# xjtu-omics/SVision

Hardware: AMD Instinct MI355X
Metric: candidate SV sites/sec (encode+CNN) (higher is better)
Workload: dtype f32

## Files before the change

include/svx.h:

```cpp
#ifndef SVX_H
#define SVX_H

#include <stdint.h>
#include <stddef.h>

#ifdef __cplusplus
extern "C" {
#endif

#define SVX_VERSION 420

#define SVX_OK            0
#define SVX_EINVAL       (-1)
#define SVX_ECAPACITY    (-2)
#define SVX_ELAUNCH      (-3)

#define SVX_IMG           227
#define SVX_LAYOUT_NHWC   0
#define SVX_LAYOUT_NCHW   1

#define SVX_GAP_INS       1
#define SVX_GAP_DEL       2

#define SVX_CONV_DENSE_PCT 97
// ... 44 lines not shown
int svx_fc_bias_act(const float* d_x, const float* d_w_packed, const float* d_bias, float* d_out, float* d_ws,
                    uint32_t m, uint32_t n, uint32_t k, int relu, void* stream);

int svx_fc8_softmax(const float* d_x, const float* d_w, const float* d_bias, float* d_out, uint32_t n, void* stream);

int svx_conv2d_same(const float* d_in, const float* d_w_packed, const float* d_bias, float* d_out, uint32_t n,
                    uint32_t cin, uint32_t cout, uint32_t height, uint32_t width, uint32_t ksize,
                    uint32_t groups, int relu, const int32_t* d_pixels, const uint32_t* d_pixel_count,
                    const float* d_background, void* stream);

int svx_image_dedup(const int32_t* d_records, uint32_t n, int32_t* d_unique, uint32_t* d_inv, uint32_t* d_live,
                    uint32_t* d_keys, uint32_t* d_ws, void* stream);

int svx_gather_rows(const float* d_src, const uint32_t* d_inv, float* d_dst, uint32_t n, uint32_t width, void* stream);

int svx_encode_conv1_live(const int32_t* d_records, uint32_t n, const float* d_w1, const float* d_base, float* d_y,
                          int lrn, uint32_t radius, float alpha, float beta, float k, uint32_t* d_touched,
                          const uint32_t* d_live, void* stream);
int svx_alexnet_active_sets_live(const uint32_t* d_touched, uint32_t n, int32_t* d_list2, int32_t* d_list3,
                                 int32_t* d_list4, int32_t* d_list5, uint32_t* d_counts, uint32_t* d_ws,
                                 uint64_t* d_totals, uint32_t* d_active2, const uint32_t* d_live, void* stream);
int svx_conv2d_same_live(const float* d_in, const float* d_w_packed, const float* d_bias, float* d_out, uint32_t n,
                         uint32_t cin, uint32_t cout, uint32_t height, uint32_t width, uint32_t ksize,
                         uint32_t groups, int relu, const int32_t* d_pixels, const uint32_t* d_pixel_count,
                         const float* d_background, const uint32_t* d_live, void* stream);
int svx_bias_relu_pool_lrn_live(const float* d_x, const float* d_bias, float* d_y, uint32_t n, uint32_t channels,
                                uint32_t height, uint32_t width, int lrn, uint32_t radius, float alpha, float beta,
                                float k, const uint32_t* d_active_rows, const float* d_background,
                                const uint32_t* d_live, void* stream);
int svx_fc_bias_act_live(const float* d_x, const float* d_w_packed, const float* d_bias, float* d_out, float* d_ws,
                         uint32_t m, uint32_t n, uint32_t k, int relu, const uint32_t* d_live, void* stream);
int svx_fc8_softmax_live(const float* d_x, const float* d_w, const float* d_bias, float* d_out, uint32_t n,
                         const uint32_t* d_live, void* stream);

int svx_span_position_distance(const double* d_start, const double* d_end, const uint64_t* d_part_off,
                               uint32_t n_parts, const uint64_t* d_out_off, uint64_t total_pairs,
                               double normalizer, double* d_out, void* stream);

typedef struct SvxHashJob {
    uint64_t x_off, y_off;
    uint32_t x_len, y_len;
    uint64_t table_off;
    uint32_t table_slots;
    uint32_t hit_cap;
    uint64_t hit_off;
} SvxHashJob;
int svx_hash_seeds(const uint8_t* d_bases, const SvxHashJob* d_jobs, uint32_t n_jobs, uint64_t* d_table,
                   int32_t* d_hits, uint32_t* d_counts, uint32_t k, uint32_t window, uint32_t max_x_len, void* stream);
int svx_hash_pack_hits(const SvxHashJob* d_jobs, uint32_t n_jobs, const int32_t* d_hits, const uint32_t* d_counts,
                       uint32_t* d_row_off, int32_t* d_packed, uint64_t packed_cap, void* stream);
size_t svx_hash_seeds_long_ws_bytes(uint32_t x_len, uint32_t y_len);
int svx_hash_seeds_long(const uint8_t* d_bases, const SvxHashJob* d_jobs, uint32_t n_jobs, uint64_t* d_table,
                        int32_t* d_hits, uint32_t* d_counts, void* d_ws, const uint64_t* d_ws_off,
                        uint32_t k, uint32_t window, uint32_t max_x_len, void* stream);

#define SVX_BAM_KEEP_SEQ 1
void*          svx_bam_open(const char* path, int threads, int flags);
void*          svx_bam_open_range(const char* path, int threads, int flags, uint64_t voff_beg, uint64_t voff_end);
const char*    svx_bam_error(void);
void           svx_bam_sizes(void* handle, uint64_t* sizes);
void           svx_bam_export(void* handle, int threads, int32_t* tid, int32_t* pos, uint16_t* flag, uint8_t* mapq,
                              int32_t* l_seq, int32_t* name_id, int64_t* cig_off, uint32_t* cigar, char* names,
                              char* header, char* ref_names, int32_t* ref_lens, int64_t* seq_off);
const uint8_t* svx_bam_seq(void* handle);
void           svx_bam_close(void* handle);

// ... 73 lines not shown
```

svision_amd/_lib.py:

```python
import ctypes
import os

_HERE = os.path.dirname(os.path.abspath(__file__))
LIB_PATH = os.path.join(_HERE, "libsvx.so")

SVX_OK = 0
SVX_EINVAL = -1
SVX_ECAPACITY = -2
SVX_ELAUNCH = -3
LAYOUT_NHWC = 0
LAYOUT_NCHW = 1
IMG = 227
GAP_INS = 1
GAP_DEL = 2

_vp, _u32, _i32, _u64, _sz = ctypes.c_void_p, ctypes.c_uint32, ctypes.c_int32, ctypes.c_uint64, ctypes.c_size_t
SYMBOLS = {
    "svx_version": (ctypes.c_int, []),
    "svx_strerror": (ctypes.c_char_p, [ctypes.c_int]),
    "svx_crc32c": (_u32, [_vp, _sz]),
    "svx_cigar_scan_ws_bytes": (_sz, [_u32, _u64]),
    "svx_cigar_scan": (ctypes.c_int, [_vp, _vp, _vp, _u32, _u64, _i32, _vp, _u64, _vp, _vp, _vp, _u64, _u32, _vp]),
    "svx_rasterize": (ctypes.c_int, [_vp, _u32, _vp, ctypes.c_int, ctypes.POINTER(ctypes.c_float), _vp]),
    "svx_encode_conv1": (ctypes.c_int, [_vp, _u32, _vp, _vp, _vp, ctypes.c_int, _u32, ctypes.c_float, ctypes.c_float,
                                        ctypes.c_float, _vp, _vp]),
    "svx_alexnet_active_sets": (ctypes.c_int, [_vp, _u32, _vp, _vp, _vp, _vp, _vp, _vp, _vp, _vp, _vp]),
    "svx_conv2d_same": (ctypes.c_int, [_vp, _vp, _vp, _vp, _u32, _u32, _u32, _u32, _u32, _u32, _u32, ctypes.c_int, _vp, _vp, _vp, _vp]),
    "svx_fc_ws_bytes": (_sz, [_u32, _u32, _u32]),
    "svx_fc_bias_act": (ctypes.c_int, [_vp, _vp, _vp, _vp, _vp, _u32, _u32, _u32, ctypes.c_int, _vp]),
    "svx_fc8_softmax": (ctypes.c_int, [_vp, _vp, _vp, _vp, _u32, _vp]),
    "svx_bias_relu_pool_lrn": (ctypes.c_int, [_vp, _vp, _vp, _u32, _u32, _u32, _u32, ctypes.c_int, _u32,
                                              ctypes.c_float, ctypes.c_float, ctypes.c_float, _vp, _vp, _vp]),
    "svx_image_dedup": (ctypes.c_int, [_vp, _u32, _vp, _vp, _vp, _vp, _vp, _vp]),
    "svx_gather_rows": (ctypes.c_int, [_vp, _vp, _vp, _u32, _u32, _vp]),
    "svx_encode_conv1_live": (ctypes.c_int, [_vp, _u32, _vp, _vp, _vp, ctypes.c_int, _u32, ctypes.c_float, ctypes.c_float,
                                             ctypes.c_float, _vp, _vp, _vp]),
    "svx_alexnet_active_sets_live": (ctypes.c_int, [_vp, _u32, _vp, _vp, _vp, _vp, _vp, _vp, _vp, _vp, _vp, _vp]),
    "svx_conv2d_same_live": (ctypes.c_int, [_vp, _vp, _vp, _vp, _u32, _u32, _u32, _u32, _u32, _u32, _u32, ctypes.c_int, _vp, _vp, _vp,
                                            _vp, _vp]),
    "svx_bias_relu_pool_lrn_live": (ctypes.c_int, [_vp, _vp, _vp, _u32, _u32, _u32, _u32, ctypes.c_int, _u32,
                                                   ctypes.c_float, ctypes.c_float, ctypes.c_float, _vp, _vp, _vp, _vp]),
    "svx_fc_bias_act_live": (ctypes.c_int, [_vp, _vp, _vp, _vp, _vp, _u32, _u32, _u32, ctypes.c_int, _vp, _vp]),
    "svx_fc8_softmax_live": (ctypes.c_int, [_vp, _vp, _vp, _vp, _u32, _vp, _vp]),
    "svx_span_position_distance":(ctypes.c_int, [_vp, _vp, _vp, _u32, _vp, _u64, ctypes.c_double, _vp, _vp]),
    "svx_hash_seeds": (ctypes.c_int, [_vp, _vp, _u32, _vp, _vp, _vp, _u32, _u32, _u32, _vp]),
    "svx_hash_pack_hits": (ctypes.c_int, [_vp, _u32, _vp, _vp, _vp, _vp, _u64, _vp]),
    "svx_hash_seeds_long_ws_bytes": (_sz, [_u32, _u32]),
    "svx_hash_seeds_long": (ctypes.c_int, [_vp, _vp, _u32, _vp, _vp, _vp, _vp, _vp, _u32, _u32, _u32, _vp]),
    "svx_bam_open": (_vp, [ctypes.c_char_p, ctypes.c_int, ctypes.c_int]),
    "svx_bam_open_range": (_vp, [ctypes.c_char_p, ctypes.c_int, ctypes.c_int, _u64, _u64]),
    "svx_bam_error": (ctypes.c_char_p, []),
    "svx_bam_sizes": (None, [_vp, _vp]),
    "svx_bam_export": (None, [_vp, ctypes.c_int] + [_vp] * 13),
    "svx_bam_seq": (_vp, [_vp]),
    "svx_bam_close": (None, [_vp]),
    "svx_bgzf_inflate_fast_ws_bytes": (_sz, [_u64, _u32]),
    "svx_bgzf_inflate_fast": (ctypes.c_int, [_vp, _vp, _vp, _vp, _u32, _u64, _vp, _vp, _vp, _u64, _vp]),
    "svx_bgzf_inflate_fast_on": (ctypes.c_int, [_vp, _vp, _vp, _vp, _u32, _u64, _vp, _vp, _vp, _u64, _vp, _vp]),
    "svx_bgzf_crc32": (ctypes.c_int, [_vp, _vp, _vp, _vp, _vp, _u32, _vp, _vp]),
    "svx_bam_walk_count": (ctypes.c_int, [_vp, _vp, _u32, _vp, _vp]),
    "svx_bam_walk_extract": (ctypes.c_int, [_vp, _vp, _u32, _vp] + [_vp] * 9 + [_u32, _vp]),
    "svx_bam_walk_count_seq": (ctypes.c_int, [_vp, _vp, _u32, _vp, _vp, _vp]),
    "svx_bam_walk_extract_seq": (ctypes.c_int, [_vp, _vp, _u32, _vp] + [_vp] * 12 + [_u32, _vp]),
    "svx_bam_find_starts_ws_bytes": (_sz, [_u32]),
    "svx_bam_find_starts": (ctypes.c_int, [_vp, _vp, _u32, _u64, _u32, _vp, _vp, _vp, _vp, _u64, _vp]),
    "svx_bam_walk_offsets": (ctypes.c_int, [_vp, _vp, _u32, _vp, _vp, _vp]),
    "svx_record_sort_ws_bytes": (_sz, [_u32]),
    "svx_record_sort": (ctypes.c_int, [_vp, _vp, _u32, _u32, _u32, _vp, _vp, _u64, _vp]),
    "svx_record_gather": (ctypes.c_int, [_vp, _vp, _vp, _u32, _u32, _vp]),
    "svx_record_gather_offsets_ws_bytes": (_sz, [_u32]),
    "svx_record_gather_offsets": (ctypes.c_int, [_vp, _vp, _u32, _vp, _vp, _u64, _vp]),
    "svx_record_gather_segments": (ctypes.c_int, [_vp, _vp, _vp, _vp, _vp, _u32, _u32, _vp]),
    "svx_record_invert": (ctypes.c_int, [_vp, _u32, _vp, _vp]),
    "svx_record_scatter_segments": (ctypes.c_int, [_vp, _vp, _vp, _u32, _u32, _vp, ctypes.c_int64, _vp, _u32, _vp, _vp]),
    "svx_bgzf_deflate": (ctypes.c_int, [_vp, _vp, _u32, _vp, _vp, _vp, _vp]),
    "svx_bgzf_deflate_dyn_ws_bytes": (_sz, [_u32]),
# ... 61 lines not shown
```

svision_amd/csrc/svx_cnn.hip:

```cpp
#include "svx_raster_common.hpp"

namespace {

constexpr int BLOCK = 256, WAVE = 64;

__device__ inline float lrn_scale(float v, float x, float beta)
{
    if (beta == 0.75f) return v * __frsqrt_rn(x) * __frsqrt_rn(__fsqrt_rn(x));
    return v / powf(x, beta);
}

__device__ inline float4 max4(float4 a, float4 b) { return make_float4(fmaxf(a.x, b.x), fmaxf(a.y, b.y), fmaxf(a.z, b.z), fmaxf(a.w, b.w)); }

__global__ __launch_bounds__(BLOCK)
void bias_relu_pool_lrn_kernel(const float* __restrict__ x, const float* __restrict__ bias, float* __restrict__ y,
                               int C, int H, int W, int OH, int OW, int lrn, int radius, float alpha, float beta, float k,
                               const uint32_t* __restrict__ active_rows, const float* __restrict__ background,
                               const uint32_t* __restrict__ live)
{
    extern __shared__ __attribute__((aligned(16))) float pooled[];
    const int b = blockIdx.x / OH;
    if (live && (uint32_t)b >= *live) return;
    const int oy = blockIdx.x - b * OH;
    const int CP = C + 1, HW = H * W;
// ... 350 lines not shown
    for (int p = t; p < 3 * A2 * A2; p += BLOCK) {
        const int l = p / (A2 * A2), q = p - l * (A2 * A2);
        const int y = q / A2, x = q - y * A2, r = A1 + l * A2 + y;
        const uint32_t m = masks[r], below = (1u << x) - 1u;
        const uint32_t slot = ((m >> x) & 1u) ? rowoff[r] + __popc(m & below) : inoff[r] + __popc(~m & below);
        ls[l][slot] = (int32_t)(img * (A2 * A2) + q);
    }
}
}

extern "C" int svx_alexnet_active_sets_live(const uint32_t* d_touched, uint32_t n, int32_t* d_list2, int32_t* d_list3,
                                            int32_t* d_list4, int32_t* d_list5, uint32_t* d_counts, uint32_t* d_ws,
                                            uint64_t* d_totals, uint32_t* d_active2, const uint32_t* d_live, void* stream)
{
    if (!d_counts) return SVX_EINVAL;
    hipStream_t st = static_cast<hipStream_t>(stream);
    if (n == 0) return hipMemsetAsync(d_counts, 0, 4 * sizeof(uint32_t), st) == hipSuccess ? SVX_OK : SVX_ELAUNCH;
    if (!d_touched || !d_list2 || !d_list3 || !d_list4 || !d_list5 || !d_ws || (reinterpret_cast<uintptr_t>(d_ws) & 15u)) return SVX_EINVAL;
    hipLaunchKernelGGL(active_counts_kernel, dim3(n), dim3(64), 0, st, d_touched, d_ws, d_live);
    hipLaunchKernelGGL(active_lists_kernel, dim3(n), dim3(BLOCK), 0, st, d_touched, d_ws, n, d_list2, d_list3, d_list4, d_list5, d_counts,
                       reinterpret_cast<unsigned long long*>(d_totals), d_active2, d_live);
    return hipGetLastError() == hipSuccess ? SVX_OK : SVX_ELAUNCH;
}

extern "C" int svx_alexnet_active_sets(const uint32_t* d_touched, uint32_t n, int32_t* d_list2, int32_t* d_list3,
                                       int32_t* d_list4, int32_t* d_list5, uint32_t* d_counts, uint32_t* d_ws,
                                       uint64_t* d_totals, uint32_t* d_active2, void* stream)
{
    return svx_alexnet_active_sets_live(d_touched, n, d_list2, d_list3, d_list4, d_list5, d_counts, d_ws, d_totals, d_active2, nullptr, stream);
}

namespace {
constexpr int FC8_IN = 4096, FC8_OUT = 5;
__global__ __launch_bounds__(64 * FC8_OUT)
void fc8_softmax_kernel(const float* __restrict__ x, const float* __restrict__ w, const float* __restrict__ bias,
                        float* __restrict__ out, const uint32_t* __restrict__ live)
{
    __shared__ float logit[FC8_OUT];
    const int img = blockIdx.x, cls = threadIdx.x >> 6, lane = threadIdx.x & 63;
    if (live && (uint32_t)img >= *live) return;
    const float4* xv = reinterpret_cast<const float4*>(x + (size_t)img * FC8_IN);
    const float4* wv = reinterpret_cast<const float4*>(w + (size_t)cls * FC8_IN);
    float acc = 0.0f;
#pragma unroll 4
    for (int i = lane; i < FC8_IN / 4; i += 64) {
        const float4 a = xv[i], b = wv[i];
        acc = fmaf(a.x, b.x, acc); acc = fmaf(a.y, b.y, acc); acc = fmaf(a.z, b.z, acc); acc = fmaf(a.w, b.w, acc);
    }
#pragma unroll
    for (int o = 32; o > 0; o >>= 1) acc += __shfl_xor(acc, o, 64);
    if (lane == 0) logit[cls] = acc + bias[cls];
    __syncthreads();
    if (threadIdx.x == 0) {
        float m = logit[0];
        int best = 0;
        for (int j = 1; j < FC8_OUT; ++j) if (logit[j] > m) { m = logit[j]; best = j; }
        float e[FC8_OUT], s = 0.0f;
        for (int j = 0; j < FC8_OUT; ++j) { e[j] = expf(logit[j] - m); s += e[j]; }
        float* o = out + (size_t)img * 12;
        for (int j = 0; j < FC8_OUT; ++j) { o[j] = e[j] / s; o[6 + j] = logit[j]; }
        o[5] = (float)best;
        o[11] = 0.0f;
    }
}
}

extern "C" int svx_fc8_softmax_live(const float* d_x, const float* d_w, const float* d_bias, float* d_out, uint32_t n,
                                    const uint32_t* d_live, void* stream)
{
    if (n == 0) return SVX_OK;
    if (!d_x || !d_w || !d_bias || !d_out) return SVX_EINVAL;
    if ((reinterpret_cast<uintptr_t>(d_x) & 15u) || (reinterpret_cast<uintptr_t>(d_w) & 15u)) return SVX_EINVAL;
    hipLaunchKernelGGL(fc8_softmax_kernel, dim3(n), dim3(64 * FC8_OUT), 0, static_cast<hipStream_t>(stream), d_x, d_w, d_bias, d_out, d_live);
    return hipGetLastError() == hipSuccess ? SVX_OK : SVX_ELAUNCH;
}

extern "C" int svx_fc8_softmax(const float* d_x, const float* d_w, const float* d_bias, float* d_out, uint32_t n, void* stream)
{
    return svx_fc8_softmax_live(d_x, d_w, d_bias, d_out, n, nullptr, stream);
}

extern "C" int svx_bias_relu_pool_lrn_live(const float* d_x, const float* d_bias, float* d_y, uint32_t n, uint32_t channels,
                                           uint32_t height, uint32_t width, int lrn, uint32_t radius, float alpha, float beta,
                                           float k, const uint32_t* d_active_rows, const float* d_background,
                                           const uint32_t* d_live, void* stream)
{
    if (n == 0) return SVX_OK;
    if (!d_x || !d_bias || !d_y || channels == 0 || channels % 8 || height < 3 || width < 3) return SVX_EINVAL;
    if ((reinterpret_cast<uintptr_t>(d_x) | reinterpret_cast<uintptr_t>(d_bias) | reinterpret_cast<uintptr_t>(d_y)) & 15u) return SVX_EINVAL;
    if ((d_active_rows == nullptr) != (d_background == nullptr) || (reinterpret_cast<uintptr_t>(d_background) & 15u) || (d_active_rows && width > 32)) return SVX_EINVAL;
    const int OH = (int)(height - 3) / 2 + 1, OW = (int)(width - 3) / 2 + 1;
    const size_t lds = (size_t)(channels + 1) * OW * sizeof(float);
    if (lds > 64 * 1024) return SVX_EINVAL;
    hipLaunchKernelGGL(bias_relu_pool_lrn_kernel, dim3(n * OH), dim3(BLOCK), lds, static_cast<hipStream_t>(stream),
                       d_x, d_bias, d_y, (int)channels, (int)height, (int)width, OH, OW, lrn, (int)radius, alpha, beta, k,
                       d_active_rows, d_background, d_live);
    return hipGetLastError() == hipSuccess ? SVX_OK : SVX_ELAUNCH;
// ... 10 lines not shown
```

svision_amd/csrc/svx_dedup.hip:

```cpp
#include "svx_raster_common.hpp"

namespace {

constexpr int KEY_BLOCK = 256, COMPACT_BLOCK = 1024, WAVE = 64;

__device__ inline bool key_eq(const uint4& a, const uint4& b) { return a.x == b.x && a.y == b.y && a.z == b.z && a.w == b.w; }

__global__ __launch_bounds__(KEY_BLOCK)
void first_kernel(const int32_t* __restrict__ records, uint32_t n, uint32_t* __restrict__ first, uint4* __restrict__ keys)
{
    __shared__ uint4 tile[KEY_BLOCK];
    const uint32_t i = blockIdx.x * KEY_BLOCK + threadIdx.x;
    const uint4 mine = i < n ? svx_raster::image_key(records + (size_t)i * 12) : uint4{0, 0, 0, 0};
    if (keys && i < n) keys[i] = mine;
    uint32_t f = i;
    for (uint32_t t = 0; t <= blockIdx.x; ++t) {
        const uint32_t j0 = t * KEY_BLOCK;
        __syncthreads();
        if (t == blockIdx.x) tile[threadIdx.x] = mine;
        else tile[threadIdx.x] = svx_raster::image_key(records + (size_t)(j0 + threadIdx.x) * 12);
        __syncthreads();
        if (f == i) {
            const uint32_t hi = min((uint32_t)KEY_BLOCK, i - j0);
            for (uint32_t j = 0; j < hi; ++j)
                if (key_eq(tile[j], mine)) { f = j0 + j; break; }
        }
    }
    if (i < n) first[i] = f;
}

__global__ __launch_bounds__(COMPACT_BLOCK)
void compact_kernel(const int32_t* __restrict__ records, uint32_t n, uint32_t* __restrict__ inv, uint32_t* __restrict__ row,
                    int32_t* __restrict__ unique, uint32_t* __restrict__ live)
{
    __shared__ uint32_t wave_sum[COMPACT_BLOCK / WAVE];
    __shared__ uint32_t s_base;
    const int t = threadIdx.x, lane = t & (WAVE - 1), wv = t / WAVE;
    if (t == 0) s_base = 0;
    __syncthreads();
    for (uint32_t c0 = 0; c0 < n; c0 += COMPACT_BLOCK) {
        const uint32_t i = c0 + t;
        const bool is_first = i < n && inv[i] == i;
        const unsigned long long ball = __ballot(is_first);
        const uint32_t below = __popcll(ball & ((1ull << lane) - 1ull));
        if (lane == 0) wave_sum[wv] = __popcll(ball);
        __syncthreads();
        uint32_t before = s_base;
        for (int w = 0; w < wv; ++w) before += wave_sum[w];
        if (is_first) {
            const uint32_t c = before + below;
            row[i] = c;
#pragma unroll
            for (int e = 0; e < 12; ++e) unique[(size_t)c * 12 + e] = records[(size_t)i * 12 + e];
        }
        __syncthreads();
        if (t == 0) { uint32_t s = s_base; for (int w = 0; w < COMPACT_BLOCK / WAVE; ++w) s += wave_sum[w]; s_base = s; }
        __syncthreads();
    }
    const uint32_t n_live = s_base;
    for (uint32_t e = n_live * 12 + t; e < n * 12; e += COMPACT_BLOCK) unique[e] = records[e % 12];
    for (uint32_t i = t; i < n; i += COMPACT_BLOCK) inv[i] = row[inv[i]];
    if (t == 0) *live = n_live;
}

__global__ __launch_bounds__(256)
void gather_rows_kernel(const float* __restrict__ src, const uint32_t* __restrict__ inv, float* __restrict__ dst, uint32_t n, uint32_t width)
{
    const uint32_t e = blockIdx.x * 256 + threadIdx.x;
    if (e >= n * width) return;
    const uint32_t i = e / width, c = e - i * width;
    dst[e] = src[(size_t)inv[i] * width + c];
}

}

extern "C" int svx_image_dedup(const int32_t* d_records, uint32_t n, int32_t* d_unique, uint32_t* d_inv, uint32_t* d_live,
                               uint32_t* d_keys, uint32_t* d_ws, void* stream)
{
    if (!d_live) return SVX_EINVAL;
    hipStream_t st = static_cast<hipStream_t>(stream);
    if (n == 0) return hipMemsetAsync(d_live, 0, sizeof(uint32_t), st) == hipSuccess ? SVX_OK : SVX_ELAUNCH;
    if (!d_records || !d_unique || !d_inv || !d_ws || n > (1u << 26)) return SVX_EINVAL;
    if (reinterpret_cast<uintptr_t>(d_keys) & 15u) return SVX_EINVAL;
    hipLaunchKernelGGL(first_kernel, dim3((n + KEY_BLOCK - 1) / KEY_BLOCK), dim3(KEY_BLOCK), 0, st, d_records, n, d_inv,
                       reinterpret_cast<uint4*>(d_keys));
    hipLaunchKernelGGL(compact_kernel, dim3(1), dim3(COMPACT_BLOCK), 0, st, d_records, n, d_inv, d_ws, d_unique, d_live);
    return hipGetLastError() == hipSuccess ? SVX_OK : SVX_ELAUNCH;
}

extern "C" int svx_gather_rows(const float* d_src, const uint32_t* d_inv, float* d_dst, uint32_t n, uint32_t width, void* stream)
{
    if (n == 0 || width == 0) return SVX_OK;
    if (!d_src || !d_inv || !d_dst || (uint64_t)n * width > 0xffffffffull) return SVX_EINVAL;
    const uint32_t total = n * width;
    hipLaunchKernelGGL(gather_rows_kernel, dim3((total + 255) / 256), dim3(256), 0, static_cast<hipStream_t>(stream), d_src, d_inv, d_dst, n, width);
    return hipGetLastError() == hipSuccess ? SVX_OK : SVX_ELAUNCH;
}
```

svision_amd/csrc/svx_fc.hip:

```cpp
#include <hip/hip_runtime.h>
#include <stdint.h>
#include "../../include/svx.h"
#include "svx_shadow.hpp"

namespace {

typedef float v16f __attribute__((ext_vector_type(16)));
typedef float v4f __attribute__((ext_vector_type(4)));
constexpr int THREADS = 256, WAVES = THREADS / 64;

__device__ __forceinline__ v4f buf_load4(__amdgpu_buffer_rsrc_t rsrc, unsigned voff, unsigned soff)
{
    return __builtin_bit_cast(v4f, __builtin_amdgcn_raw_buffer_load_b128(rsrc, (int)voff, (int)soff, 0));
}

#ifndef SVX_FC_RING_A
#define SVX_FC_RING_A 6
#endif

template <int U> struct StageIndex { static constexpr int value = U; };

template <int N, int U = 0, typename F>
__device__ __forceinline__ void svx_unroll_stages(F& f)
{
    if constexpr (U < N) { f(StageIndex<U>{}); svx_unroll_stages<N, U + 1>(f); }
}

template <int N, int U = 0, typename F>
__device__ __forceinline__ void svx_tail_stages(F& f, int left)
{
    if constexpr (U < N - 1) {
        if (left > U) { f(StageIndex<U>{}); svx_tail_stages<N, U + 1>(f, left); }
    }
}

struct FcArgs { const float* x; const float* w; float* part; int M, N, K, splits; const uint32_t* live; };

template <int NA, int NB>
__global__ __launch_bounds__(THREADS, 2)
void fc_splitk_kernel(const FcArgs a)
{
    SVX_SHADOW_ROOM();
    const int n_tiles = a.N / (32 * NA), m_tiles = (a.M + 32 * NB - 1) / (32 * NB);
    const int total = m_tiles * a.splits * n_tiles;
    const int wt = blockIdx.x * WAVES + (threadIdx.x >> 6);
    if (wt >= total) return;
    const int nt = wt % n_tiles, rest = wt / n_tiles;
    const int s = rest % a.splits, mt = rest / a.splits;
    const int m_live = a.live ? min((int)*a.live, a.M) : a.M;
    if (mt * 32 * NB >= m_live) return;
    const int lane = threadIdx.x & 63, hi = lane >> 5, lo = lane & 31;
    const int KQ = a.K / 8;
    const int q0 = (int)((long long)KQ * s / a.splits), q1 = (int)((long long)KQ * (s + 1) / a.splits);
    const __amdgpu_buffer_rsrc_t rs_w = __builtin_amdgcn_make_buffer_rsrc(const_cast<float*>(a.w), 0, (int)((long long)a.N * a.K * 4), 0x00020000);
    const __amdgpu_buffer_rsrc_t rs_x = __builtin_amdgcn_make_buffer_rsrc(const_cast<float*>(a.x), 0, (int)((long long)a.M * a.K * 4), 0x00020000);
    unsigned voff_a[NA], voff_b[NB];
#pragma unroll
    for (int i = 0; i < NA; ++i) voff_a[i] = (unsigned)((((nt * NA + i) * KQ + q0) * 32 + lo) * 32 + 16 * hi);
#pragma unroll
    for (int t = 0; t < NB; ++t) voff_b[t] = (unsigned)(((mt * NB + t) * 32 + lo) * a.K * 4 + (q0 * 8 + 4 * hi) * 4);
    v16f acc[NA][NB];
#pragma unroll
    for (int i = 0; i < NA; ++i)
#pragma unroll
        for (int t = 0; t < NB; ++t)
#pragma unroll
            for (int r = 0; r < 16; ++r) acc[i][t][r] = 0.0f;
    constexpr int RA = SVX_FC_RING_A, RB = 3, MF = 4 * NA * NB, L = NA + NB;
    static_assert(RA % RB == 0, "weight ring must be a multiple of the activation ring");
    v4f ra[RA][NA], rb[RB][NB];
    unsigned soff_a = 0, soff_b = 0;
    auto load_a = [&](int slot) {
#pragma unroll
        for (int i = 0; i < NA; ++i) ra[slot][i] = buf_load4(rs_w, voff_a[i], soff_a);
        soff_a += 1024u;
    };
    auto load_b1 = [&](int slot, int t) { rb[slot][t] = buf_load4(rs_x, voff_b[t], soff_b); };
    auto stage = [&](auto u_) {
        constexpr int u = decltype(u_)::value;
        constexpr int sa = u % RA, sb = u % RB, la = (u + RA - 1) % RA, lb = (u + RB - 1) % RB;
#pragma unroll
        for (int m = 0; m < MF; ++m) {
            if (m == 0) load_a(la);
#pragma unroll
            for (int t = 0; t < NB; ++t)
                if ((t + 1) * MF / L == m) load_b1(lb, t);
            const int j = m / (NA * NB), r = m - j * (NA * NB);
            const int i = r / NB, t = r - i * NB;
            acc[i][t] = __builtin_amdgcn_mfma_f32_32x32x2f32(ra[sa][i][j], rb[sb][t][j], acc[i][t], 0, 0, 0);
            __builtin_amdgcn_sched_barrier(0);
        }
        soff_b += 32u;
    };
    const int Q = q1 - q0;
#pragma unroll
    for (int p = 0; p < RA - 1; ++p) load_a(p);
#pragma unroll
    for (int p = 0; p < RB - 1; ++p) {
#pragma unroll
        for (int t = 0; t < NB; ++t) load_b1(p, t);
        soff_b += 32u;
    }
    __builtin_amdgcn_sched_barrier(0);
    const int QU = Q - Q % RA;
    for (int q = 0; q < QU; q += RA) svx_unroll_stages<RA>(stage);
    svx_tail_stages<RA>(stage, Q - QU);
#pragma unroll
    for (int i = 0; i < NA; ++i)
#pragma unroll
        for (int t = 0; t < NB; ++t) {
            const int m = (mt * NB + t) * 32 + lo;
            if (m >= m_live) continue;
            float* o = a.part + ((size_t)s * a.M + m) * a.N + (nt * NA + i) * 32 + 4 * hi;
#pragma unroll
            for (int u = 0; u < 4; ++u)
                *reinterpret_cast<v4f*>(o + 8 * u) = v4f{acc[i][t][4 * u], acc[i][t][4 * u + 1], acc[i][t][4 * u + 2], acc[i][t][4 * u + 3]};
        }
}

__global__ __launch_bounds__(THREADS)
void fc_reduce_kernel(const float* __restrict__ part, const float* __restrict__ bias, float* __restrict__ out, int MN4, int N4, int splits, int relu,
                      const uint32_t* __restrict__ live)
{
    const int e = blockIdx.x * THREADS + threadIdx.x;
    if (e >= MN4 || (live && (uint32_t)(e / N4) >= *live)) return;
    const float4* p = reinterpret_cast<const float4*>(part);
    float4 v = reinterpret_cast<const float4*>(bias)[e % N4];
    for (int s = 0; s < splits; ++s) { const float4 q = p[(size_t)s * MN4 + e]; v.x += q.x; v.y += q.y; v.z += q.z; v.w += q.w; }
    if (relu) { v.x = fmaxf(v.x, 0.0f); v.y = fmaxf(v.y, 0.0f); v.z = fmaxf(v.z, 0.0f); v.w = fmaxf(v.w, 0.0f); }
    reinterpret_cast<float4*>(out)[e] = v;
}

int fc_na(uint32_t m, uint32_t n)
{
    int na = (m > 64 && n % 64 == 0) ? 2 : 1;
#ifdef SVX_CONV_EXPERIMENT
    if (const char* e = getenv("SVX_FC_NA")) if (atoi(e) == 1 || (atoi(e) == 2 && m > 32 && n % 64 == 0)) na = atoi(e);
#endif
    return na;
}

int fc_splits(uint32_t m, uint32_t n, uint32_t k)
{
    const int tiles = (int)(n / (32 * fc_na(m, n))) * (int)((m + 63) / 64);
    int s = (1024 + tiles - 1) / tiles;
    const int max_s = (int)(k / 8) / 24;
    if (s > max_s) s = max_s;
#ifdef SVX_CONV_EXPERIMENT
    if (const char* e = getenv("SVX_FC_SPLITS")) if (atoi(e) >= 1 && atoi(e) <= max_s) s = atoi(e);
#endif
    return s < 1 ? 1 : s;
}

}

extern "C" size_t svx_fc_ws_bytes(uint32_t m, uint32_t n, uint32_t k)
{
    return (size_t)fc_splits(m, n, k) * m * n * sizeof(float);
}

extern "C" int svx_fc_bias_act_live(const float* d_x, const float* d_w_packed, const float* d_bias, float* d_out, float* d_ws,
                                    uint32_t m, uint32_t n, uint32_t k, int relu, const uint32_t* d_live, void* stream)
{
    if (m == 0) return SVX_OK;
    if (!d_x || !d_w_packed || !d_bias || !d_out || !d_ws || n % 32 || k % 8 || k < 24 * 8) return SVX_EINVAL;
    for (const void* p : {(const void*)d_x, (const void*)d_w_packed, (const void*)d_bias, (const void*)d_out, (const void*)d_ws})
        if (reinterpret_cast<uintptr_t>(p) & 15u) return SVX_EINVAL;
    if ((uint64_t)n * k * 4 > 0x7fffffffull || (uint64_t)m * k * 4 > 0x7fffffffull) return SVX_EINVAL;
    hipStream_t st = static_cast<hipStream_t>(stream);
    FcArgs a{d_x, d_w_packed, d_ws, (int)m, (int)n, (int)k, fc_splits(m, n, k), d_live};
    const int m_tiles = (int)((m + 63) / 64);
    const int na = fc_na(m, n);
    const int waves = m_tiles * a.splits * (int)(n / (32 * na));
    const dim3 grid((unsigned)((waves + WAVES - 1) / WAVES));
    if (na == 2)      hipLaunchKernelGGL((fc_splitk_kernel<2, 2>), grid, dim3(THREADS), 0, st, a);
    else if (m <= 32) hipLaunchKernelGGL((fc_splitk_kernel<1, 1>), grid, dim3(THREADS), 0, st, a);
    else              hipLaunchKernelGGL((fc_splitk_kernel<1, 2>), grid, dim3(THREADS), 0, st, a);
    const int mn4 = (int)((uint64_t)m * n / 4);
    hipLaunchKernelGGL(fc_reduce_kernel, dim3((mn4 + THREADS - 1) / THREADS), dim3(THREADS), 0, st, d_ws, d_bias, d_out, mn4, (int)(n / 4), a.splits, relu, d_live);
    return hipGetLastError() == hipSuccess ? SVX_OK : SVX_ELAUNCH;
}

extern "C" int svx_fc_bias_act(const float* d_x, const float* d_w_packed, const float* d_bias, float* d_out, float* d_ws,
                               uint32_t m, uint32_t n, uint32_t k, int relu, void* stream)
{
    return svx_fc_bias_act_live(d_x, d_w_packed, d_bias, d_out, d_ws, m, n, k, relu, nullptr, stream);
}
```

svision_amd/kernels.py:

```python
import ctypes

import numpy as np
import torch

from . import _lib

GAP_DTYPE = np.dtype([("aln", "<u4"), ("op", "<u4"), ("read_pos", "<i4"),
                      ("ref_pos", "<i4"), ("len", "<i4"), ("kind", "<u4")])
MEAN = (104.0, 117.0, 124.0)


def to_c8(x):
    n, c, h, w = x.shape
    if c % 8:
        raise _lib.SvxError("the C8 layout needs a channel count that is a multiple of 8")
    return x.reshape(n, c // 8, 8, h, w).permute(0, 1, 3, 4, 2).contiguous()


def from_c8(x):
    n, o, h, w, e = x.shape
    return x.permute(0, 1, 4, 2, 3).reshape(n, o * e, h, w).contiguous()


def pack_conv_weights(w_hwio):
# ... 252 lines not shown
def fc_bias_act(x, w_packed, bias, relu=True, out=None, ws=None, live=None):
    lib = _lib.load()
    for t, nm in ((x, "x"), (w_packed, "w_packed"), (bias, "bias")):
        _require_cuda(t, nm)
    if x.dtype != torch.float32 or x.dim() != 2 or w_packed.dim() != 4 or w_packed.shape[2:] != (32, 8) or w_packed.shape[1] * 8 != x.shape[1]:
        raise _lib.SvxError("x must be float32 [m,k] and w packed [n/32,k/8,32,8]")
    m, k = x.shape
    n = w_packed.shape[0] * 32
    if bias.numel() != n:
        raise _lib.SvxError("bias must have n entries")
    if out is None:
        out = torch.empty((m, n), dtype=torch.float32, device=x.device)
    need = lib.svx_fc_ws_bytes(m, n, k)
    if ws is None or ws.numel() * ws.element_size() < need:
        ws = torch.empty(max(need, 16) // 4, dtype=torch.float32, device=x.device)
    rc = lib.svx_fc_bias_act_live(x.data_ptr(), w_packed.data_ptr(), bias.data_ptr(), out.data_ptr(), ws.data_ptr(), m, n, k,
                                  1 if relu else 0, _check_live(live), _stream_ptr(x.device))
    _lib.check(rc, "svx_fc_bias_act")
    return out


def fc8_softmax(x, w_out_in, bias, out=None, live=None):
    lib = _lib.load()
    for t, nm in ((x, "x"), (w_out_in, "w"), (bias, "bias")):
        _require_cuda(t, nm)
    if x.dtype != torch.float32 or x.dim() != 2 or x.shape[1] != 4096 or tuple(w_out_in.shape) != (5, 4096):
        raise _lib.SvxError("x must be float32 [n,4096] and w float32 [5,4096]")
    n = x.shape[0]
    if out is None:
        out = torch.empty((n, 12), dtype=torch.float32, device=x.device)
    rc = lib.svx_fc8_softmax_live(x.data_ptr(), w_out_in.data_ptr(), bias.data_ptr(), out.data_ptr(), n, _check_live(live),
                                  _stream_ptr(x.device))
    _lib.check(rc, "svx_fc8_softmax")
    return out


def span_position_distance(starts, ends, part_off, normalizer=1000.0):
    lib = _lib.load()
    _require_cuda(starts, "starts")
    _require_cuda(ends, "ends")
    if starts.dtype != torch.float64 or ends.dtype != torch.float64 or starts.numel() != ends.numel():
        raise _lib.SvxError("starts / ends must be float64 tensors of one length")
    part = np.ascontiguousarray(part_off, np.uint64)
    if part.ndim != 1 or part.size < 1 or int(part[-1]) != starts.numel() or np.any(np.diff(part.astype(np.int64)) < 0):
        raise _lib.SvxError("part_off must be ascending and end at the number of signatures")
    sizes = np.diff(part.astype(np.int64))
    out_off = np.zeros(part.size, np.uint64)
    out_off[1:] = np.cumsum(sizes * (sizes - 1) // 2)
    total = int(out_off[-1])
    out = torch.empty(total, dtype=torch.float64, device=starts.device)
    if total:
        d_part = torch.from_numpy(part.view(np.int64)).to(starts.device)
        d_off = torch.from_numpy(out_off.view(np.int64)).to(starts.device)
        rc = lib.svx_span_position_distance(starts.data_ptr(), ends.data_ptr(), d_part.data_ptr(), part.size - 1, d_off.data_ptr(), total,
                                            float(normalizer), out.data_ptr(), _stream_ptr(starts.device))
        _lib.check(rc, "svx_span_position_distance")
    return out, out_off


HASH_MAX_X = 2048
HASH_LONG_MAX_X = 65536
_BASE_CODE = np.full(256, 255, np.uint8)
for _i, _c in enumerate(b"ACGTNacgtnRYKMS"):
    _BASE_CODE[_c] = _i
HASH_JOB_DTYPE = np.dtype([("x_off", "<u8"), ("y_off", "<u8"), ("x_len", "<u4"), ("y_len", "<u4"), ("table_off", "<u8"),
                           ("table_slots", "<u4"), ("hit_cap", "<u4"), ("hit_off", "<u8")])
# ... 454 lines not shown
```

svision_amd/network/alexnet.py:

```python
import numpy as np
import torch

CLASSES = ("DEL", "INS", "INV", "DUP", "tDUP")

_CONVS = (
    ("conv1", 11, 3, 96, 4, 0, 1),
    ("conv2", 5, 48, 256, 1, 2, 2),
    ("conv3", 3, 256, 384, 1, 1, 1),
    ("conv4", 3, 192, 384, 1, 1, 2),
    ("conv5", 3, 192, 256, 1, 1, 2),
)
_FCS = (("fc6", 9216, 4096), ("fc7", 4096, 4096), ("fc8", 4096, 5))


def checkpoint_shapes():
    shapes = {}
    for name, k, cin, cout, _s, _p, _g in _CONVS:
        shapes[f"{name}/weights"] = (k, k, cin, cout)
        shapes[f"{name}/biases"] = (cout,)
    for name, nin, nout in _FCS:
        shapes[f"{name}/weights"] = (nin, nout)
        shapes[f"{name}/biases"] = (nout,)
    return shapes

# ... 101 lines not shown
    @torch.no_grad()
    def background(self):
        if self._background is None:
            from .. import kernels
            from .create_batch import PAD_DATA, parse_data_fields
            dev = self.conv1_base.device
            rec = torch.tensor([parse_data_fields(PAD_DATA.split("_"))], dtype=torch.int32, device=dev)
            x1, touched = kernels.encode_conv1(rec, self.conv1_hwio, self.conv1_base, touched=True)
            rows = touched[0].cpu().numpy().astype("int64") & ((1 << 27) - 1)
            free = [(y, x) for y in range(27) for x in range(27) if not (int(rows[y]) >> x) & 1]
            if not free:
                raise RuntimeError("the padding record touches every pooled pixel")
            c = x1[0, :, free[0][0], free[0][1], :]
            x = c.reshape(1, 12, 1, 1, 8).expand(1, 12, 27, 27, 8).contiguous()
            bg = {}
            bg["conv2"] = kernels.conv2d_same(x, self.conv2_w, None, groups=2)
            x = kernels.bias_relu_pool_lrn(bg["conv2"], self.conv2_b, lrn=True)
            bg["conv3"] = kernels.conv2d_same(x, self.conv3_w, self.conv3_b, groups=1, relu=True)
            bg["conv4"] = kernels.conv2d_same(bg["conv3"], self.conv4_w, self.conv4_b, groups=2, relu=True)
            bg["conv5"] = kernels.conv2d_same(bg["conv4"], self.conv5_w, None, groups=2)
            self._background = bg
        return self._background

    @torch.no_grad()
    def predict_records_packed(self, records, out=None, memo=None):
        from .. import kernels
        memo = self.memo if memo is None else bool(memo)
        live = inv = None
        if memo and records.shape[0] > 0:
            records, inv, live = kernels.image_dedup(records)
        x = self._convs(records, live)
        x = x.reshape(x.shape[0], 9216)
        x = kernels.fc_bias_act(x, self.fc6_w, self.fc6_b, relu=True, live=live)
        x = kernels.fc_bias_act(x, self.fc7_w, self.fc7_b, relu=True, live=live)
        if live is None:
            return kernels.fc8_softmax(x, self.fc8_w, self.fc8_b, out=out)
        packed = kernels.fc8_softmax(x, self.fc8_w, self.fc8_b, live=live)
        return kernels.gather_rows(packed, inv, out=out)

    @torch.no_grad()
    def predict_records(self, records):
        packed = self.predict_records_packed(records)
        return packed[:, 6:11], packed[:, 5].to(torch.int64), packed[:, :5]
```

Measured before the change: 7779.

## Fuse fc7 reduce, fc8 softmax and row gather; add small-batch dedup and live FC path

On the memoized path, fc7's split-K reduce, bias and ReLU are folded into a new fc8 tail kernel. That kernel also computes the softmax and scatters results to duplicate rows through the inverse map, which replaces three launches. Deduplication gets a single-block kernel for batches of at most one compact block, skipping the separate first-occurrence pass. The FC split-K kernel gets a live-count-aware variant that picks narrow tiles when few unique rows survive. The risks are an O(n) scan of inv per block in the tail kernel, and a quadratic key comparison in the small dedup kernel.

```diff
diff --git a/include/svx.h b/include/svx.h
--- a/include/svx.h
+++ b/include/svx.h
@@ -100,6 +100,12 @@
                          uint32_t m, uint32_t n, uint32_t k, int relu, const uint32_t* d_live, void* stream);
 int svx_fc8_softmax_live(const float* d_x, const float* d_w, const float* d_bias, float* d_out, uint32_t n,
                          const uint32_t* d_live, void* stream);
+
+uint32_t svx_fc_splits(uint32_t m, uint32_t n, uint32_t k);
+int svx_fc_partial_live(const float* d_x, const float* d_w_packed, float* d_ws, uint32_t m, uint32_t n, uint32_t k,
+                        const uint32_t* d_live, void* stream);
+int svx_fc8_tail_live(const float* d_part, uint32_t splits, const float* d_bias7, const float* d_w, const float* d_bias,
+                      const uint32_t* d_inv, float* d_out, uint32_t m, uint32_t n, const uint32_t* d_live, void* stream);
 
 int svx_span_position_distance(const double* d_start, const double* d_end, const uint64_t* d_part_off,
                                uint32_t n_parts, const uint64_t* d_out_off, uint64_t total_pairs,
diff --git a/svision_amd/_lib.py b/svision_amd/_lib.py
--- a/svision_amd/_lib.py
+++ b/svision_amd/_lib.py
@@ -42,6 +42,9 @@
                                                    ctypes.c_float, ctypes.c_float, ctypes.c_float, _vp, _vp, _vp, _vp]),
     "svx_fc_bias_act_live": (ctypes.c_int, [_vp, _vp, _vp, _vp, _vp, _u32, _u32, _u32, ctypes.c_int, _vp, _vp]),
     "svx_fc8_softmax_live": (ctypes.c_int, [_vp, _vp, _vp, _vp, _u32, _vp, _vp]),
+    "svx_fc_splits": (_u32, [_u32, _u32, _u32]),
+    "svx_fc_partial_live": (ctypes.c_int, [_vp, _vp, _vp, _u32, _u32, _u32, _vp, _vp]),
+    "svx_fc8_tail_live": (ctypes.c_int, [_vp, _u32, _vp, _vp, _vp, _vp, _vp, _u32, _u32, _vp, _vp]),
     "svx_span_position_distance":(ctypes.c_int, [_vp, _vp, _vp, _u32, _vp, _u64, ctypes.c_double, _vp, _vp]),
     "svx_hash_seeds": (ctypes.c_int, [_vp, _vp, _u32, _vp, _vp, _vp, _u32, _u32, _u32, _vp]),
     "svx_hash_pack_hits": (ctypes.c_int, [_vp, _u32, _vp, _vp, _vp, _vp, _u64, _vp]),
diff --git a/svision_amd/csrc/svx_cnn.hip b/svision_amd/csrc/svx_cnn.hip
--- a/svision_amd/csrc/svx_cnn.hip
+++ b/svision_amd/csrc/svx_cnn.hip
@@ -406,14 +406,9 @@
 
 namespace {
 constexpr int FC8_IN = 4096, FC8_OUT = 5;
-__global__ __launch_bounds__(64 * FC8_OUT)
-void fc8_softmax_kernel(const float* __restrict__ x, const float* __restrict__ w, const float* __restrict__ bias,
-                        float* __restrict__ out, const uint32_t* __restrict__ live)
-{
-    __shared__ float logit[FC8_OUT];
-    const int img = blockIdx.x, cls = threadIdx.x >> 6, lane = threadIdx.x & 63;
-    if (live && (uint32_t)img >= *live) return;
-    const float4* xv = reinterpret_cast<const float4*>(x + (size_t)img * FC8_IN);
+__device__ __forceinline__ void fc8_row(const float4* xv, const float* __restrict__ w, const float* __restrict__ bias, float* logit, float* o)
+{
+    const int cls = threadIdx.x >> 6, lane = threadIdx.x & 63;
     const float4* wv = reinterpret_cast<const float4*>(w + (size_t)cls * FC8_IN);
     float acc = 0.0f;
 #pragma unroll 4
@@ -422,7 +417,7 @@
         acc = fmaf(a.x, b.x, acc); acc = fmaf(a.y, b.y, acc); acc = fmaf(a.z, b.z, acc); acc = fmaf(a.w, b.w, acc);
     }
 #pragma unroll
-    for (int o = 32; o > 0; o >>= 1) acc += __shfl_xor(acc, o, 64);
+    for (int d = 32; d > 0; d >>= 1) acc += __shfl_xor(acc, d, 64);
     if (lane == 0) logit[cls] = acc + bias[cls];
     __syncthreads();
     if (threadIdx.x == 0) {
@@ -431,12 +426,59 @@
         for (int j = 1; j < FC8_OUT; ++j) if (logit[j] > m) { m = logit[j]; best = j; }
         float e[FC8_OUT], s = 0.0f;
         for (int j = 0; j < FC8_OUT; ++j) { e[j] = expf(logit[j] - m); s += e[j]; }
-        float* o = out + (size_t)img * 12;
         for (int j = 0; j < FC8_OUT; ++j) { o[j] = e[j] / s; o[6 + j] = logit[j]; }
         o[5] = (float)best;
         o[11] = 0.0f;
     }
 }
+
+__global__ __launch_bounds__(64 * FC8_OUT)
+void fc8_softmax_kernel(const float* __restrict__ x, const float* __restrict__ w, const float* __restrict__ bias,
+                        float* __restrict__ out, const uint32_t* __restrict__ live)
+{
+    __shared__ float logit[FC8_OUT];
+    const int img = blockIdx.x;
+    if (live && (uint32_t)img >= *live) return;
+    fc8_row(reinterpret_cast<const float4*>(x + (size_t)img * FC8_IN), w, bias, logit, out + (size_t)img * 12);
+}
+
+__global__ __launch_bounds__(64 * FC8_OUT)
+void fc8_tail_kernel(const float* __restrict__ part, const float* __restrict__ bias7, const float* __restrict__ w, const float* __restrict__ bias,
+                     const uint32_t* __restrict__ inv, float* __restrict__ out, uint32_t m, uint32_t n, int splits, const uint32_t* __restrict__ live)
+{
+    __shared__ float4 xs[FC8_IN / 4];
+    __shared__ float logit[FC8_OUT];
+    __shared__ float packed[12];
+    const uint32_t img = blockIdx.x;
+    if (live && img >= *live) return;
+    const size_t mn4 = (size_t)m * (FC8_IN / 4);
+    const float4* p = reinterpret_cast<const float4*>(part) + (size_t)img * (FC8_IN / 4);
+    for (int i = threadIdx.x; i < FC8_IN / 4; i += 64 * FC8_OUT) {
+        float4 v = reinterpret_cast<const float4*>(bias7)[i];
+        for (int s = 0; s < splits; ++s) { const float4 q = p[(size_t)s * mn4 + i]; v.x += q.x; v.y += q.y; v.z += q.z; v.w += q.w; }
+        v.x = fmaxf(v.x, 0.0f); v.y = fmaxf(v.y, 0.0f); v.z = fmaxf(v.z, 0.0f); v.w = fmaxf(v.w, 0.0f);
+        xs[i] = v;
+    }
+    __syncthreads();
+    fc8_row(xs, w, bias, logit, packed);
+    __syncthreads();
+    for (uint32_t i = threadIdx.x; i < n; i += 64 * FC8_OUT)
+        if (inv[i] == img) {
+#pragma unroll
+            for (int e = 0; e < 12; ++e) out[(size_t)i * 12 + e] = packed[e];
+        }
+}
+}
+
+extern "C" int svx_fc8_tail_live(const float* d_part, uint32_t splits, const float* d_bias7, const float* d_w, const float* d_bias,
+                                 const uint32_t* d_inv, float* d_out, uint32_t m, uint32_t n, const uint32_t* d_live, void* stream)
+{
+    if (m == 0 || n == 0) return SVX_OK;
+    if (!d_part || !d_bias7 || !d_w || !d_bias || !d_inv || !d_out || splits == 0) return SVX_EINVAL;
+    if ((reinterpret_cast<uintptr_t>(d_part) | reinterpret_cast<uintptr_t>(d_bias7) | reinterpret_cast<uintptr_t>(d_w)) & 15u) return SVX_EINVAL;
+    hipLaunchKernelGGL(fc8_tail_kernel, dim3(m), dim3(64 * FC8_OUT), 0, static_cast<hipStream_t>(stream), d_part, d_bias7, d_w, d_bias, d_inv, d_out,
+                       m, n, (int)splits, d_live);
+    return hipGetLastError() == hipSuccess ? SVX_OK : SVX_ELAUNCH;
 }
 
 extern "C" int svx_fc8_softmax_live(const float* d_x, const float* d_w, const float* d_bias, float* d_out, uint32_t n,
diff --git a/svision_amd/csrc/svx_dedup.hip b/svision_amd/csrc/svx_dedup.hip
--- a/svision_amd/csrc/svx_dedup.hip
+++ b/svision_amd/csrc/svx_dedup.hip
@@ -36,9 +36,10 @@
     __shared__ uint32_t wave_sum[COMPACT_BLOCK / WAVE];
     __shared__ uint32_t s_base;
     const int t = threadIdx.x, lane = t & (WAVE - 1), wv = t / WAVE;
+    const uint32_t block = blockDim.x;
     if (t == 0) s_base = 0;
     __syncthreads();
-    for (uint32_t c0 = 0; c0 < n; c0 += COMPACT_BLOCK) {
+    for (uint32_t c0 = 0; c0 < n; c0 += block) {
         const uint32_t i = c0 + t;
         const bool is_first = i < n && inv[i] == i;
         const unsigned long long ball = __ballot(is_first);
@@ -54,13 +55,54 @@
             for (int e = 0; e < 12; ++e) unique[(size_t)c * 12 + e] = records[(size_t)i * 12 + e];
         }
         __syncthreads();
-        if (t == 0) { uint32_t s = s_base; for (int w = 0; w < COMPACT_BLOCK / WAVE; ++w) s += wave_sum[w]; s_base = s; }
+        if (t == 0) { uint32_t s = s_base; for (uint32_t w = 0; w < block / WAVE; ++w) s += wave_sum[w]; s_base = s; }
         __syncthreads();
     }
     const uint32_t n_live = s_base;
-    for (uint32_t e = n_live * 12 + t; e < n * 12; e += COMPACT_BLOCK) unique[e] = records[e % 12];
-    for (uint32_t i = t; i < n; i += COMPACT_BLOCK) inv[i] = row[inv[i]];
+    for (uint32_t e = n_live * 12 + t; e < n * 12; e += block) unique[e] = records[e % 12];
+    for (uint32_t i = t; i < n; i += block) inv[i] = row[inv[i]];
     if (t == 0) *live = n_live;
+}
+
+__global__ __launch_bounds__(COMPACT_BLOCK)
+void dedup_small_kernel(const int32_t* __restrict__ records, uint32_t n, uint32_t* __restrict__ inv, int32_t* __restrict__ unique,
+                        uint32_t* __restrict__ live, uint4* __restrict__ keys)
+{
+    constexpr uint32_t SCAN = 8;
+    __shared__ uint4 tile[COMPACT_BLOCK];
+    __shared__ uint32_t row[COMPACT_BLOCK];
+    __shared__ uint32_t wave_sum[COMPACT_BLOCK / WAVE];
+    const uint32_t i = threadIdx.x, lane = i & (WAVE - 1), wv = i / WAVE, block = blockDim.x;
+    const uint4 mine = i < n ? svx_raster::image_key(records + (size_t)i * 12) : uint4{0, 0, 0, 0};
+    if (keys && i < n) keys[i] = mine;
+    tile[i] = mine;
+    __syncthreads();
+    uint32_t f = i;
+    if (i < n)
+        for (uint32_t j0 = 0; j0 < i && f == i; j0 += SCAN) {
+            uint32_t hit = 0;
+#pragma unroll
+            for (uint32_t u = 0; u < SCAN; ++u)
+                if (key_eq(tile[j0 + u], mine) && j0 + u < i) hit |= 1u << u;
+            if (hit) f = j0 + __ffs(hit) - 1;
+        }
+    const bool is_first = i < n && f == i;
+    const unsigned long long ball = __ballot(is_first);
+    const uint32_t below = __popcll(ball & ((1ull << lane) - 1ull));
+    if (lane == 0) wave_sum[wv] = __popcll(ball);
+    __syncthreads();
+    uint32_t before = 0, n_live = 0;
+    for (uint32_t w = 0; w < block / WAVE; ++w) { if (w == wv) before = n_live; n_live += wave_sum[w]; }
+    if (is_first) {
+        const uint32_t c = before + below;
+        row[i] = c;
+#pragma unroll
+        for (int e = 0; e < 12; ++e) unique[(size_t)c * 12 + e] = records[(size_t)i * 12 + e];
+    }
+    __syncthreads();
+    if (i < n) inv[i] = row[f];
+    for (uint32_t e = n_live * 12 + i; e < n * 12; e += block) unique[e] = records[e % 12];
+    if (i == 0) *live = n_live;
 }
 
 __global__ __launch_bounds__(256)
@@ -82,9 +124,14 @@
     if (n == 0) return hipMemsetAsync(d_live, 0, sizeof(uint32_t), st) == hipSuccess ? SVX_OK : SVX_ELAUNCH;
     if (!d_records || !d_unique || !d_inv || !d_ws || n > (1u << 26)) return SVX_EINVAL;
     if (reinterpret_cast<uintptr_t>(d_keys) & 15u) return SVX_EINVAL;
+    const uint32_t block = n >= COMPACT_BLOCK ? COMPACT_BLOCK : (n + WAVE - 1) / WAVE * WAVE;
+    if (n <= COMPACT_BLOCK) {
+        hipLaunchKernelGGL(dedup_small_kernel, dim3(1), dim3(block), 0, st, d_records, n, d_inv, d_unique, d_live, reinterpret_cast<uint4*>(d_keys));
+        return hipGetLastError() == hipSuccess ? SVX_OK : SVX_ELAUNCH;
+    }
     hipLaunchKernelGGL(first_kernel, dim3((n + KEY_BLOCK - 1) / KEY_BLOCK), dim3(KEY_BLOCK), 0, st, d_records, n, d_inv,
                        reinterpret_cast<uint4*>(d_keys));
-    hipLaunchKernelGGL(compact_kernel, dim3(1), dim3(COMPACT_BLOCK), 0, st, d_records, n, d_inv, d_ws, d_unique, d_live);
+    hipLaunchKernelGGL(compact_kernel, dim3(1), dim3(block), 0, st, d_records, n, d_inv, d_ws, d_unique, d_live);
     return hipGetLastError() == hipSuccess ? SVX_OK : SVX_ELAUNCH;
 }
 
diff --git a/svision_amd/csrc/svx_fc.hip b/svision_amd/csrc/svx_fc.hip
--- a/svision_amd/csrc/svx_fc.hip
+++ b/svision_amd/csrc/svx_fc.hip
@@ -17,6 +17,9 @@
 #ifndef SVX_FC_RING_A
 #define SVX_FC_RING_A 6
 #endif
+#ifndef SVX_FC_RING_NARROW
+#define SVX_FC_RING_NARROW 6
+#endif
 
 template <int U> struct StageIndex { static constexpr int value = U; };
 
@@ -36,19 +39,9 @@
 
 struct FcArgs { const float* x; const float* w; float* part; int M, N, K, splits; const uint32_t* live; };
 
-template <int NA, int NB>
-__global__ __launch_bounds__(THREADS, 2)
-void fc_splitk_kernel(const FcArgs a)
-{
-    SVX_SHADOW_ROOM();
-    const int n_tiles = a.N / (32 * NA), m_tiles = (a.M + 32 * NB - 1) / (32 * NB);
-    const int total = m_tiles * a.splits * n_tiles;
-    const int wt = blockIdx.x * WAVES + (threadIdx.x >> 6);
-    if (wt >= total) return;
-    const int nt = wt % n_tiles, rest = wt / n_tiles;
-    const int s = rest % a.splits, mt = rest / a.splits;
-    const int m_live = a.live ? min((int)*a.live, a.M) : a.M;
-    if (mt * 32 * NB >= m_live) return;
+template <int NA, int NB, int RA>
+__device__ __forceinline__ void fc_tile(const FcArgs& a, int nt, int s, int mt, int m_live)
+{
     const int lane = threadIdx.x & 63, hi = lane >> 5, lo = lane & 31;
     const int KQ = a.K / 8;
     const int q0 = (int)((long long)KQ * s / a.splits), q1 = (int)((long long)KQ * (s + 1) / a.splits);
@@ -66,7 +59,7 @@
         for (int t = 0; t < NB; ++t)
 #pragma unroll
             for (int r = 0; r < 16; ++r) acc[i][t][r] = 0.0f;
-    constexpr int RA = SVX_FC_RING_A, RB = 3, MF = 4 * NA * NB, L = NA + NB;
+    constexpr int RB = 3, MF = 4 * NA * NB, L = NA + NB;
     static_assert(RA % RB == 0, "weight ring must be a multiple of the activation ring");
     v4f ra[RA][NA], rb[RB][NB];
     unsigned soff_a = 0, soff_b = 0;
@@ -118,6 +111,47 @@
         }
 }
 
+template <int NA, int NB>
+__global__ __launch_bounds__(THREADS, 2)
+void fc_splitk_kernel(const FcArgs a)
+{
+    SVX_SHADOW_ROOM();
+    const int n_tiles = a.N / (32 * NA), m_tiles = (a.M + 32 * NB - 1) / (32 * NB);
+    const int total = m_tiles * a.splits * n_tiles;
+    const int wt = blockIdx.x * WAVES + (threadIdx.x >> 6);
+    if (wt >= total) return;
+    const int nt = wt % n_tiles, rest = wt / n_tiles;
+    const int s = rest % a.splits, mt = rest / a.splits;
+    const int m_live = a.live ? min((int)*a.live, a.M) : a.M;
+    if (mt * 32 * NB >= m_live) return;
+    fc_tile<NA, NB, SVX_FC_RING_A>(a, nt, s, mt, m_live);
+}
+
+template <int NA>
+__global__ __launch_bounds__(THREADS, 2)
+void fc_splitk_live_kernel(const FcArgs a)
+{
+    SVX_SHADOW_ROOM();
+    const int m_live = min((int)*a.live, a.M);
+    const int wv = threadIdx.x >> 6;
+    if (m_live > 64) {
+        const int n_tiles = a.N / (32 * NA), m_tiles = (a.M + 63) / 64;
+        const int wt = blockIdx.x * WAVES + wv;
+        if (wt >= m_tiles * a.splits * n_tiles) return;
+        const int nt = wt % n_tiles, rest = wt / n_tiles;
+        const int s = rest % a.splits, mt = rest / a.splits;
+        if (mt * 64 >= m_live) return;
+        fc_tile<NA, 2, SVX_FC_RING_A>(a, nt, s, mt, m_live);
+        return;
+    }
+    if (m_live == 0) return;
+    const int n_tiles = a.N / 32;
+    const int pair = m_live > 32 ? 1 : 0;
+    const int item = (int)(blockIdx.x + (wv >> pair) * gridDim.x);
+    if (item >= n_tiles * a.splits) return;
+    fc_tile<1, 1, SVX_FC_RING_NARROW>(a, item % n_tiles, item / n_tiles, pair ? (wv & 1) : 0, m_live);
+}
+
 __global__ __launch_bounds__(THREADS)
 void fc_reduce_kernel(const float* __restrict__ part, const float* __restrict__ bias, float* __restrict__ out, int MN4, int N4, int splits, int relu,
                       const uint32_t* __restrict__ live)
@@ -159,12 +193,17 @@
     return (size_t)fc_splits(m, n, k) * m * n * sizeof(float);
 }
 
-extern "C" int svx_fc_bias_act_live(const float* d_x, const float* d_w_packed, const float* d_bias, float* d_out, float* d_ws,
-                                    uint32_t m, uint32_t n, uint32_t k, int relu, const uint32_t* d_live, void* stream)
+extern "C" uint32_t svx_fc_splits(uint32_t m, uint32_t n, uint32_t k)
+{
+    return (uint32_t)fc_splits(m, n, k);
+}
+
+extern "C" int svx_fc_partial_live(const float* d_x, const float* d_w_packed, float* d_ws, uint32_t m, uint32_t n, uint32_t k,
+                                   const uint32_t* d_live, void* stream)
 {
     if (m == 0) return SVX_OK;
-    if (!d_x || !d_w_packed || !d_bias || !d_out || !d_ws || n % 32 || k % 8 || k < 24 * 8) return SVX_EINVAL;
-    for (const void* p : {(const void*)d_x, (const void*)d_w_packed, (const void*)d_bias, (const void*)d_out, (const void*)d_ws})
+    if (!d_x || !d_w_packed || !d_ws || n % 32 || k % 8 || k < 24 * 8) return SVX_EINVAL;
+    for (const void* p : {(const void*)d_x, (const void*)d_w_packed, (const void*)d_ws})
         if (reinterpret_cast<uintptr_t>(p) & 15u) return SVX_EINVAL;
     if ((uint64_t)n * k * 4 > 0x7fffffffull || (uint64_t)m * k * 4 > 0x7fffffffull) return SVX_EINVAL;
     hipStream_t st = static_cast<hipStream_t>(stream);
@@ -172,12 +211,30 @@
     const int m_tiles = (int)((m + 63) / 64);
     const int na = fc_na(m, n);
     const int waves = m_tiles * a.splits * (int)(n / (32 * na));
+    if (d_live && m > 64) {
+        const int items = a.splits * (int)(n / 32);
+        const dim3 grid((unsigned)(((waves > 2 * items ? waves : 2 * items) + WAVES - 1) / WAVES));
+        if (na == 2) hipLaunchKernelGGL((fc_splitk_live_kernel<2>), grid, dim3(THREADS), 0, st, a);
+        else         hipLaunchKernelGGL((fc_splitk_live_kernel<1>), grid, dim3(THREADS), 0, st, a);
+        return hipGetLastError() == hipSuccess ? SVX_OK : SVX_ELAUNCH;
+    }
     const dim3 grid((unsigned)((waves + WAVES - 1) / WAVES));
     if (na == 2)      hipLaunchKernelGGL((fc_splitk_kernel<2, 2>), grid, dim3(THREADS), 0, st, a);
     else if (m <= 32) hipLaunchKernelGGL((fc_splitk_kernel<1, 1>), grid, dim3(THREADS), 0, st, a);
     else              hipLaunchKernelGGL((fc_splitk_kernel<1, 2>), grid, dim3(THREADS), 0, st, a);
+    return hipGetLastError() == hipSuccess ? SVX_OK : SVX_ELAUNCH;
+}
+
+extern "C" int svx_fc_bias_act_live(const float* d_x, const float* d_w_packed, const float* d_bias, float* d_out, float* d_ws,
+                                    uint32_t m, uint32_t n, uint32_t k, int relu, const uint32_t* d_live, void* stream)
+{
+    if (m == 0) return SVX_OK;
+    if (!d_bias || !d_out || (reinterpret_cast<uintptr_t>(d_bias) & 15u) || (reinterpret_cast<uintptr_t>(d_out) & 15u)) return SVX_EINVAL;
+    const int rc = svx_fc_partial_live(d_x, d_w_packed, d_ws, m, n, k, d_live, stream);
+    if (rc != SVX_OK) return rc;
     const int mn4 = (int)((uint64_t)m * n / 4);
-    hipLaunchKernelGGL(fc_reduce_kernel, dim3((mn4 + THREADS - 1) / THREADS), dim3(THREADS), 0, st, d_ws, d_bias, d_out, mn4, (int)(n / 4), a.splits, relu, d_live);
+    hipLaunchKernelGGL(fc_reduce_kernel, dim3((mn4 + THREADS - 1) / THREADS), dim3(THREADS), 0, static_cast<hipStream_t>(stream), d_ws, d_bias, d_out,
+                       mn4, (int)(n / 4), fc_splits(m, n, k), relu, d_live);
     return hipGetLastError() == hipSuccess ? SVX_OK : SVX_ELAUNCH;
 }
 
diff --git a/svision_amd/kernels.py b/svision_amd/kernels.py
--- a/svision_amd/kernels.py
+++ b/svision_amd/kernels.py
@@ -308,6 +308,38 @@
     rc = lib.svx_fc8_softmax_live(x.data_ptr(), w_out_in.data_ptr(), bias.data_ptr(), out.data_ptr(), n, _check_live(live),
                                   _stream_ptr(x.device))
     _lib.check(rc, "svx_fc8_softmax")
+    return out
+
+
+def fc_partial(x, w_packed, live=None):
+    lib = _lib.load()
+    for t, nm in ((x, "x"), (w_packed, "w_packed")):
+        _require_cuda(t, nm)
+    if x.dtype != torch.float32 or x.dim() != 2 or w_packed.dim() != 4 or w_packed.shape[2:] != (32, 8) or w_packed.shape[1] * 8 != x.shape[1]:
+        raise _lib.SvxError("x must be float32 [m,k] and w packed [n/32,k/8,32,8]")
+    m, k = x.shape
+    n = w_packed.shape[0] * 32
+    part = torch.empty((lib.svx_fc_splits(m, n, k), m, n), dtype=torch.float32, device=x.device)
+    rc = lib.svx_fc_partial_live(x.data_ptr(), w_packed.data_ptr(), part.data_ptr(), m, n, k, _check_live(live), _stream_ptr(x.device))
+    _lib.check(rc, "svx_fc_partial")
+    return part
+
+
+def fc8_tail(part, bias7, w_out_in, bias, inv, out=None, live=None):
+    lib = _lib.load()
+    for t, nm in ((part, "part"), (bias7, "bias7"), (w_out_in, "w"), (bias, "bias"), (inv, "inv")):
+        _require_cuda(t, nm)
+    if part.dtype != torch.float32 or part.dim() != 3 or part.shape[2] != 4096 or not part.is_contiguous() or bias7.numel() != 4096 \
+            or tuple(w_out_in.shape) != (5, 4096) or inv.dtype != torch.int32 or inv.dim() != 1:
+        raise _lib.SvxError("part must be a contiguous float32 [splits,m,4096], bias7 [4096], w float32 [5,4096] and inv int32 [n]")
+    splits, m, n = part.shape[0], part.shape[1], inv.shape[0]
+    if out is None:
+        out = torch.empty((n, 12), dtype=torch.float32, device=part.device)
+    elif tuple(out.shape) != (n, 12) or out.dtype != torch.float32 or not out.is_contiguous():
+        raise _lib.SvxError("out must be a contiguous float32 [n,12] tensor")
+    rc = lib.svx_fc8_tail_live(part.data_ptr(), splits, bias7.data_ptr(), w_out_in.data_ptr(), bias.data_ptr(), inv.data_ptr(),
+                               out.data_ptr(), m, n, _check_live(live), _stream_ptr(part.device))
+    _lib.check(rc, "svx_fc8_tail")
     return out
 
 
diff --git a/svision_amd/network/alexnet.py b/svision_amd/network/alexnet.py
--- a/svision_amd/network/alexnet.py
+++ b/svision_amd/network/alexnet.py
@@ -157,11 +157,11 @@
         x = self._convs(records, live)
         x = x.reshape(x.shape[0], 9216)
         x = kernels.fc_bias_act(x, self.fc6_w, self.fc6_b, relu=True, live=live)
-        x = kernels.fc_bias_act(x, self.fc7_w, self.fc7_b, relu=True, live=live)
         if live is None:
+            x = kernels.fc_bias_act(x, self.fc7_w, self.fc7_b, relu=True)
             return kernels.fc8_softmax(x, self.fc8_w, self.fc8_b, out=out)
-        packed = kernels.fc8_softmax(x, self.fc8_w, self.fc8_b, live=live)
-        return kernels.gather_rows(packed, inv, out=out)
+        part = kernels.fc_partial(x, self.fc7_w, live=live)
+        return kernels.fc8_tail(part, self.fc7_b, self.fc8_w, self.fc8_b, inv, out=out, live=live)
 
     @torch.no_grad()
     def predict_records(self, records):
```

After: 8062 (median of 6 runs). 3.6% higher.
